# iyioon/NYPC-Yacht-Auction

Hardware: AMD Instinct MI355X
Metric: MCTS node-expansions/sec/GPU @4096 envs x100 sims; episodes/sec 1-8 GPU (higher is better)
Workload: dtype f32

## Files before the change

### include/yacht_hip.h

```cpp
#ifndef YACHT_HIP_H
#define YACHT_HIP_H

#include <stdint.h>

#ifdef __cplusplus
extern "C" {
#endif

#define YK_ACTION_SIZE 3226
#define YK_NUM_BID_ACTIONS 202
#define YK_FEATURES 59
#define YK_MASK_WORDS 101

typedef struct { uint64_t w[8]; } yk_state_t;

#define YK_OK 0
#define YK_ERR_ARG (-1)
#define YK_ERR_HIP (-2)
#define YK_ERR_NOMEM (-3)
#define YK_ERR_CAPACITY (-4)
#define YK_ERR_STATE (-5)
#define YK_ERR_RANGE (-6)

#define YK_ST_OK 0
// ... 64 lines not shown
                       void* stream);

typedef struct {
    int n_envs;
    int sims;
    double cpuct;
    int temp_threshold;
    int max_moves;
    int prior;
    int record_predictions;
    int max_expansions;
    int64_t arena_entries;
    int record_stride;
    int groups;
    int dual_trees;
    double dirichlet_alpha;
    double dirichlet_eps;
    int record_root_values;
} yk_engine_config_t;

typedef struct yk_engine yk_engine_t;
int yk_engine_create(yk_engine_t** eng, const yk_engine_config_t* cfg, yk_net_t* net);
int yk_engine_destroy(yk_engine_t* eng);
int yk_selfplay(yk_engine_t* eng, uint64_t seed, uint32_t env_base, void* stream);
int yk_engine_profile(yk_engine_t* eng, int enable);
int yk_engine_kernel_times(yk_engine_t* eng, double* ms, int64_t* launches);
int yk_engine_stats(yk_engine_t* eng, int64_t* out);
int yk_engine_counters(yk_engine_t* eng, int64_t* out, int n);
int yk_engine_records(yk_engine_t* eng, uint64_t* states, int32_t* info, uint64_t* ctr, double* values,
                      uint64_t* final_states, int32_t* n_moves, int64_t* visits_off, int32_t* visits,
                      int64_t* n_visits);
int yk_engine_predictions(yk_engine_t* eng, float* pi, float* v, yk_state_t* leaves, int32_t* count);
int yk_engine_root_priors(yk_engine_t* eng, float* before, float* after);
int yk_dirichlet_noise(uint64_t seed, const uint32_t* env_ids, const int32_t* moves, const int32_t* nvalid,
                       double alpha, double* eta, int n, void* stream);
int64_t yk_engine_record_bytes(yk_engine_t* eng);
int yk_engine_pack_records(yk_engine_t* eng, void* dst, int64_t capacity, void* stream);

int yk_examples_from_records(const void* images, int n_images, int n_envs, int max_moves, int sims,
                             int64_t n_games, int64_t skip, int64_t capacity, yk_state_t* states, int32_t* targets,
                             float* values, int64_t* n_examples, void* stream);
int yk_examples_policies(const void* images, int n_images, int n_envs, int max_moves, int sims, int64_t n_games,
                         int64_t skip, int64_t n_examples, int64_t* pi_indptr, int32_t* pi_cols, double* pi_vals,
                         int64_t nnz_capacity, double* values, int64_t* nnz, void* stream);
int yk_examples_value_targets(const void* images, int n_images, int n_envs, int max_moves, int sims,
                              int64_t n_games, int64_t skip, int64_t n_examples, double beta, double lambda,
                              float* values, float* root_values, int64_t* n_missing, void* stream);
#define YK_SYM_CARRY 1
#define YK_SYM_ROLLS 2
#define YK_SYM_GROUPS 4
int yk_examples_augment(const yk_state_t* states, const int32_t* targets, const int64_t* pi_indptr,
                        const int32_t* pi_cols, const double* pi_vals, int64_t n, int64_t index_base, uint64_t seed,
                        uint32_t epoch_key, int flags, yk_state_t* out_states, int32_t* out_targets,
                        int32_t* out_cols, double* out_vals, void* stream);

#define YK_PLAYER_MCTS 0
#define YK_PLAYER_RANDOM 1
#define YK_PLAYER_GREEDY 2
int yk_arena(yk_engine_t* eng, uint64_t seed, uint32_t env_base, const int32_t* agent_seat, int agent, int opponent,
             void* stream);
int yk_engine_set_opponent_net(yk_engine_t* eng, yk_net_t* net);
int yk_arena_results(yk_engine_t* eng, double* result, int32_t* totals, int32_t* n_moves, int32_t* actions,
                     uint64_t* final_states, uint64_t* rng_ctr);

int yk_mcts_search(yk_engine_t* eng, const yk_state_t* roots, uint64_t seed, const uint32_t* env_ids,
                   uint64_t* rng_ctr, int sims, int32_t* counts, void* stream);
// ... 44 lines not shown
```

### nypc-yacht-auction_amd/csrc/yk_engine.hip

```cpp
#include <math.h>

#include <algorithm>
#include <vector>

#include "yk_api.h"
#include "yk_common.h"
#include "yk_engine_dev.h"
#include "yk_net.h"

#define YK_MAX_GROUPS 8

using namespace yk;

namespace {


struct PwPlan {
    int nleaf, nop, root;
    uint16_t start[64], len[64];
    uint8_t a[64], b[64];
};
constexpr int pw_build(PwPlan& p, int start, int n) {
    if (n <= 128) {
        p.start[p.nleaf] = (uint16_t)start;
// ... 18 lines not shown
constexpr bool plan_is_butterfly() {
    const PwPlan p = make_plan();
    if (p.nleaf != 32 || p.nop != 31) return false;
    int first[128] = {}, cnt[128] = {};
    for (int i = 0; i < p.nleaf; i++) {
        if (p.start[i] % 8 != 0 || p.len[i] < 8 || p.len[i] > 128) return false;
        if (i > 0 && p.start[i] != p.start[i - 1] + p.len[i - 1]) return false;
        first[i] = i;
        cnt[i] = 1;
    }
    for (int o = 0; o < p.nop; o++) {
        const int a = p.a[o], b = p.b[o];
        if (cnt[a] != cnt[b] || first[a] + cnt[a] != first[b] || first[a] % (2 * cnt[a]) != 0) return false;
        first[64 + o] = first[a];
        cnt[64 + o] = 2 * cnt[a];
    }
    return p.root == 64 + p.nop - 1 && cnt[p.root] == 32;
}
static_assert(plan_is_butterfly(), "numpy's pairwise tree for 3226 is no longer a perfect 32-leaf tree");
constexpr int pw_gmax() {
    const PwPlan p = make_plan();
    int g = 0;
    for (int i = 0; i < p.nleaf; i++) g = p.len[i] / 8 > g ? p.len[i] / 8 : g;
    return g;
}
constexpr int pw_tmax() {
    const PwPlan p = make_plan();
    int t = 0;
    for (int i = 0; i < p.nleaf; i++) t = p.len[i] % 8 > t ? p.len[i] % 8 : t;
    return t;
}
constexpr int PW_GMAX = pw_gmax();
constexpr int PW_TMAX = pw_tmax() > 0 ? pw_tmax() : 1;

struct ValidQ {
    int mode;
    int n;
    uint32_t used;
    __device__ __forceinline__ bool operator()(int a) const {
        if (mode == 1) return a < NBID;
        if (mode != 0 || a < NBID) return false;
        const int base = a - NBID, cat = base / NCOMB, ci = base - cat * NCOMB;
        if ((used >> cat) & 1u) return false;
        if (n >= 10) return true;
        if (n == 5) return ci == 0;
        return c_tab.comb_max[ci] < n;
    }
};
__device__ __forceinline__ ValidQ valid_q(const YkS& s) {
    ValidQ q;
    const int round = s_round(s), phase = s_phase(s);
    const uint64_t wa = s_pw(s, 0, 0);
    q.n = __builtin_amdgcn_readfirstlane(wa_n(wa));
    q.used = __builtin_amdgcn_readfirstlane((uint32_t)wa_used(wa));
    q.mode = __builtin_amdgcn_readfirstlane((phase == 0 && round != 13) ? 1 : (phase == 1 && q.n >= 5) ? 0 : -1);
    return q;
}


__device__ __forceinline__ void wave_sync() {
    __builtin_amdgcn_fence(__ATOMIC_ACQ_REL, "workgroup");
    __builtin_amdgcn_wave_barrier();
}

__device__ __forceinline__ float wave_max(float v) {
    v = fmaxf(v, xlane<32>(v));
// ... 462 lines not shown
    const int t = __builtin_amdgcn_readfirstlane(tree_of(d, e));
    const int g = __builtin_amdgcn_readfirstlane((int)d.gen[t]);
    const bool idle = d.idle[e] != 0;
    expand_backup_game(d, e, lane, t, g);
    if (do_select) {
        if (idle) {
            select_none(d, e, lane);
            return;
        }
        wave_sync();
        select_game(d, e, lane, t, g, env_ids, ctr_arr);
    }
}

__device__ __forceinline__ void expand_backup_game(const EngDev& d, int e, int lane, int t, int g) {
    PyV res{d.res_v[e], d.res_t[e]};
    uint32_t end_id = 0;
    if (d.leaf_flag[e]) {
        const YkS s = ld_state(d.leaf_state + e);
        const uint64_t ihsh = d.leaf_hash[e];
        const uint64_t hsh = d.prior == 1 ? key_hash(s) : 0ull;
        const VInfo vi = valid_info(s, 1);
        const ValidQ valid = valid_q(s);
        const int V = vi.V;
        const int leaf = lane >> 1, h = lane & 1;
        const int st = c_pw.start[leaf], nl = c_pw.len[leaf], G = nl >> 3, R = nl & 7;
        float4 q[PW_GMAX];
        float qt[PW_TMAX];
        float v, mx = 0.f, lse = 0.f;
        const int pidx = (int)d.gstats[(long)e * GST + 0];
        const bool rec = d.rec_pred && (e % d.rec_stride) == 0 && pidx < d.max_exp;
        const long rslot = rec ? (long)(e / d.rec_stride) * d.max_exp + pidx : 0;
        bool masked = false;
        if (d.prior == 0) {
            const float* x = d.logits + (long)e * PI_LD + st;
            const float2 ml = d.mlse[e];
            mx = ml.x;
            lse = ml.y;
            if (d.fparts > 1) {
                float ms = ml.y;
                for (int p = 1; p < d.fparts; p++) {
                    const float2 q = d.mlse[(long)p * d.E + e];
                    const float mm = fmaxf(mx, q.x);
                    if (mm != -INFINITY) {
                        ms = ms * exp_acc(mx - mm) + q.y * exp_acc(q.x - mm);
                        mx = mm;
                    }
                }
                lse = logf(ms);
            }
            static_assert(NBID % 4 == 2 && NCOMB % 4 == 0, "category starts are 2 mod 4");
            const bool score10 = valid.mode == 0 && valid.n >= 10;
#pragma unroll
            for (int j = 0; j < PW_GMAX; j++) {
                const int a = st + 8 * j + 4 * h;
                bool v0, v1, v2, v3;
                if (score10) {
                    const int b0 = a - NBID, b2 = a + 2 - NBID;
                    const bool lo = j < G && b0 >= 0 && !((valid.used >> ((unsigned)b0 / NCOMB)) & 1u);
                    const bool hi = j < G && b2 >= 0 && !((valid.used >> ((unsigned)b2 / NCOMB)) & 1u);
                    v0 = v1 = lo;
                    v2 = v3 = hi;
                } else {
                    v0 = j < G && valid(a);
                    v1 = j < G && valid(a + 1);
                    v2 = j < G && valid(a + 2);
                    v3 = j < G && valid(a + 3);
                }
                float4 x4 = make_float4(0.f, 0.f, 0.f, 0.f);
                if (v0 || v1 || v2 || v3) x4 = *reinterpret_cast<const float4*>(x + 8 * j + 4 * h);
                q[j] = make_float4(v0 ? softmax_p(x4.x, mx, lse) : 0.f, v1 ? softmax_p(x4.y, mx, lse) : 0.f,
                                   v2 ? softmax_p(x4.z, mx, lse) : 0.f, v3 ? softmax_p(x4.w, mx, lse) : 0.f);
            }
#pragma unroll
            for (int r = 0; r < PW_TMAX; r++)
                qt[r] = (h == 0 && r < R && valid(st + 8 * G + r)) ? softmax_p(x[8 * G + r], mx, lse) : 0.f;
            v = d.vpred[e];
            masked = true;
        } else {
#pragma unroll
            for (int j = 0; j < PW_GMAX; j++) {
                const int a = st + 8 * j + 4 * h;
                q[j] = j < G ? make_float4(hash_prior_pi(hsh, a), hash_prior_pi(hsh, a + 1), hash_prior_pi(hsh, a + 2),
                                           hash_prior_pi(hsh, a + 3))
                             : make_float4(0.f, 0.f, 0.f, 0.f);
            }
#pragma unroll
            for (int r = 0; r < PW_TMAX; r++) qt[r] = (h == 0 && r < R) ? hash_prior_pi(hsh, st + 8 * G + r) : 0.f;
            v = hash_prior_v(hsh);
        }
#pragma unroll
        for (int j = 0; j < PW_GMAX; j++) {
            const int a = st + 8 * j + 4 * h;
            if (j < G && !masked) {
                if (!valid(a)) q[j].x = 0.f;
                if (!valid(a + 1)) q[j].y = 0.f;
                if (!valid(a + 2)) q[j].z = 0.f;
                if (!valid(a + 3)) q[j].w = 0.f;
            }
        }
#pragma unroll
        for (int r = 0; r < PW_TMAX; r++)
            if (h == 0 && r < R && !masked && !valid(st + 8 * G + r)) qt[r] = 0.f;
        if (rec) {
            float* rpi = d.rec_pi + rslot * ASIZE;
#pragma unroll
            for (int j = 0; j < PW_GMAX; j++)
                if (j < G) *reinterpret_cast<float4*>(rpi + st + 8 * j + 4 * h) = q[j];
#pragma unroll
            for (int r = 0; r < PW_TMAX; r++)
                if (h == 0 && r < R) rpi[st + 8 * G + r] = qt[r];
            if (lane == 0) {
                d.rec_v[rslot] = v;
                st_state(d.rec_leaf + rslot, s);
            }
        }
        float4 racc = q[0];
#pragma unroll
        for (int j = 1; j < PW_GMAX; j++)
            if (j < G) {
                racc.x += q[j].x;
                racc.y += q[j].y;
// ... 15 lines not shown
        lsum = (lane & 8) ? y + lsum : lsum + y;
        y = xlane<16>(lsum);
        lsum = (lane & 16) ? y + lsum : lsum + y;
        y = xlane<32>(lsum);
        lsum = (lane & 32) ? y + lsum : lsum + y;
        const float sum = lsum;
        const int VP = pad4(V);
        const uint32_t off = d.arena_top[t];
        const uint32_t nid = d.node_count[g * d.T + t];
        bool ok = true;
        if ((int64_t)off + VP > d.AE) {
            if (lane == 0) atomicOr(d.err, ERR_ARENA);
            ok = false;
        }
        if (nid >= (uint32_t)d.NCAP) {
            if (lane == 0) atomicOr(d.err, ERR_NODES);
            ok = false;
        }
        if (ok) {
            float* P = d.arenaP + (long)t * d.AE + off;
            uint16_t* S = d.arenaS + (long)t * d.AE + off;
            const float inv_fallback = V > 0 ? 1.0f / (float)V : 0.0f;
            const float* __restrict__ xr = d.logits + (long)e * PI_LD;
            const float sqe0 = (float)sqrt((double)0u + 1e-8);
            float fb = -INFINITY;
            int fj = 0x7FFFFFFF;
            for (int j0 = lane; j0 < VP; j0 += 256) {
                float xa[4];
                int aa[4];
#pragma unroll
                for (int u = 0; u < 4; u++) {
                    const int j = j0 + 64 * u;
                    aa[u] = j < V ? compact_to_action(vi, j) : 0;
                    xa[u] = (d.prior == 0 && j < V) ? xr[aa[u]] : 0.f;
                }
#pragma unroll
                for (int u = 0; u < 4; u++) {
                    const int j = j0 + 64 * u;
                    if (j < VP) {
                        float p = 0.0f;
                        if (j < V) {
                            const float pa = d.prior == 0 ? softmax_p(xa[u], mx, lse) : hash_prior_pi(hsh, aa[u]);
                            p = sum > 0.0f ? pa / sum : inv_fallback;
                            const float u0 = (d.c32 * p) * sqe0;
                            if (u0 > fb) {
                                fb = u0;
                                fj = j;
                            }
                        }
                        P[j] = p;
                        S[j] = 0;
                    }
                }
            }
            wave_argmax_step(fb, fj);
            if (lane == 0) {
                NodeRec r;
#pragma unroll
                for (int i = 0; i < 8; i++) r.key[i] = s.w[i];
                r.hash = ihsh;
                r.vinfo = pack_vinfo(vi);
                r.p_off = off;
                r.nvalid = (uint32_t)V;
                r.Ns = 0;
                r.first_j = (uint32_t)fj;
                d.nodes[g][(long)t * d.NCAP + nid] = r;
                if (!insert_index(d, g, t, ihsh, nid)) atomicOr(d.err, ERR_HASH);
            }
            end_id = nid + 1;
            if (lane == 0) {
                d.node_count[g * d.T + t] = nid + 1;
                d.arena_top[t] = off + (uint32_t)VP;
                unsigned long long* gs = reinterpret_cast<unsigned long long*>(d.gstats + (long)e * GST);
                atomicAdd(gs + 0, 1ull);
                atomicAdd(gs + 3, (unsigned long long)V);
                atomicMax(gs + 4, (unsigned long long)(nid + 1));
                atomicMax(gs + 6, (unsigned long long)(off + (uint32_t)VP));
            }
        }
        res = PyV{-(double)v, T_F32};
    } else {
        end_id = d.end_node[e];
    }
    const int depth = d.path_len[e];
    if (depth > 0) {
        NodeRec* nodes = d.nodes[g] + (long)t * d.NCAP;
        Edge* edges = d.edges[g] + (long)t * d.ECAP;
        uint16_t* Sb = d.arenaS + (long)t * d.AE;
        const uint64_t* path = d.path + (long)e * MAXD;
        const uint32_t ne0 = d.edge_count[g * d.T + t];
        uint64_t pe = 0;
        uint16_t sl = 0;
        if (lane < depth) {
            pe = path[lane];
            sl = Sb[pe >> 32];
        }
        const uint32_t pnext = __shfl((uint32_t)pe, (lane + 1) & 63, 64);
        const uint32_t cnode = lane + 1 < depth ? (pnext & ~PATH_DET) + 1 : end_id;
        const uint32_t cbits = ((uint32_t)pe & PATH_DET) ? cnode << 2 : 0u;
        const bool is_new = lane < depth && sl == 0;
        const uint64_t bal = __ballot(is_new);
        const uint32_t eid = ne0 + (uint32_t)__popcll(bal & ((1ull << lane) - 1));
        const uint32_t ne1 = ne0 + (uint32_t)__popcll(bal);
        if (lane < depth) {
            PyV v = res;
            if ((depth - 1 - lane) & 1) v.v = -v.v;
            if (sl) {
                Edge& ed = edges[sl - 1];
// ... 651 lines not shown
    A(d.idle, E);
    A(d.gstats, E * GST);
    A(d.err, 1);
    A(eng->done_count, 1);
    A(eng->mcts_env, E);
    if (d.prior == 0) {
        A(eng->logits, E * (size_t)PI_LD);
    }
    eng->root_values = cfg->record_root_values != 0;
    eng->noise = cfg->dirichlet_alpha > 0.0 && cfg->dirichlet_eps > 0.0;
    eng->nz.alpha = cfg->dirichlet_alpha;
    eng->nz.eps = cfg->dirichlet_eps;
    if (eng->noise) {
        A(eng->nz.noised, E);
        if (d.rec_pred) {
            A(eng->nz.prior_before, R * (size_t)d.M * ASIZE);
            A(eng->nz.prior_after, R * (size_t)d.M * ASIZE);
        }
    }
    if (d.rec_pred) {
        A(d.rec_pi, R * (size_t)d.max_exp * ASIZE);
        A(d.rec_v, R * (size_t)d.max_exp);
        A(d.rec_leaf, R * (size_t)d.max_exp);
    }
#undef A
    if (hipHostMalloc((void**)&eng->host_done, sizeof(int32_t)) != hipSuccess) return YK_ERR_NOMEM;
    {
        const char* ev = getenv("YK_ROOT_SCAN");
        eng->root_scan = !(ev && ev[0] == '0');
        const char* ek = getenv("YK_ROOT_K");
        d.ro_k = ek ? std::max(1, std::min(RO_K, atoi(ek))) : RO_K;
        const char* en = getenv("YK_NODE_SUMMARY");
        d.node_summary = (en && en[0] == '0') ? 0 : 1;
        const char* es = getenv("YK_SPLIT_DESCENT");
        eng->split_descent = es && es[0] == '1';
    }
    if (G > 1) {
        if (hipEventCreateWithFlags(&eng->ev_fork, hipEventDisableTiming) != hipSuccess) return YK_ERR_HIP;
        for (int g = 0; g < G; g++)
            if (hipStreamCreateWithFlags(&eng->gs[g], hipStreamNonBlocking) != hipSuccess ||
                hipEventCreateWithFlags(&eng->ev_join[g], hipEventDisableTiming) != hipSuccess ||
                hipEventCreateWithFlags(&eng->ev_fwd[g], hipEventDisableTiming) != hipSuccess)
                return YK_ERR_HIP;
    }
    if (eng->fparts_dual > 0) {
        if (hipStreamCreateWithFlags(&eng->dstream, hipStreamNonBlocking) != hipSuccess ||
            hipEventCreateWithFlags(&eng->ev_d0, hipEventDisableTiming) != hipSuccess ||
            hipEventCreateWithFlags(&eng->ev_d1, hipEventDisableTiming) != hipSuccess)
            return YK_ERR_HIP;
    }
    d.logits = eng->logits;
    d.vpred = eng->vpred;
    d.mlse = eng->mlse;
    d.lut_sq = eng->lut_sq;
    d.lut_sqe = eng->lut_sqe;
    hipLaunchKernelGGL(k_lut, dim3(LUT_N / 256), dim3(256), 0, 0, eng->lut_sq, eng->lut_sqe);
    YK_LAUNCHED();
    YK_HIP(hipMemset(d.err, 0, sizeof(uint32_t)));
    YK_HIP(hipMemset(d.done, 0, E));
    YK_HIP(hipMemset(d.idle, 0, E));
    YK_HIP(hipMemset(d.leaf_state, 0, sizeof(yk_state_t) * E));
    std::vector<uint32_t> ids(E);
    for (size_t i = 0; i < E; i++) ids[i] = (uint32_t)i;
    YK_HIP(hipMemcpy(eng->mcts_env, ids.data(), sizeof(uint32_t) * E, hipMemcpyHostToDevice));
    YK_HIP(hipDeviceSynchronize());
    *out = eng.release();
// ... 179 lines not shown
    YK_HIP(hipDeviceSynchronize());
    YK_HIP(hipMemcpy(gs.data(), d.gstats, sizeof(uint64_t) * gs.size(), hipMemcpyDeviceToHost));
    YK_HIP(hipMemcpy(nm.data(), d.nmoves, sizeof(int32_t) * nm.size(), hipMemcpyDeviceToHost));
    YK_HIP(hipMemcpy(&err, d.err, sizeof(uint32_t), hipMemcpyDeviceToHost));
    for (int i = 0; i < 16; i++) out[i] = 0;
    for (int e = 0; e < d.E; e++) {
        const uint64_t* g = &gs[(size_t)e * GST];
        out[0] += (int64_t)g[0];
        out[1] += (int64_t)g[1];
        out[2] = std::max<int64_t>(out[2], nm[e]);
        out[4] = std::max<int64_t>(out[4], (int64_t)g[4]);
        out[5] = std::max<int64_t>(out[5], (int64_t)g[5]);
        out[6] = std::max<int64_t>(out[6], (int64_t)g[6]);
        out[7] += (int64_t)g[3];
        out[8] += (int64_t)g[2];
        out[9] = std::max<int64_t>(out[9], (int64_t)g[7]);
    }
    out[3] = err;
    out[10] = d.NCAP;
    out[11] = d.ECAP;
    out[12] = d.AE;
    out[13] = d.VCAP;
    out[14] = eng->ngroups;
    out[15] = d.fparts;
    return YK_OK;
}

int yk_engine_counters(yk_engine_t* eng, int64_t* out, int n) {
    if (!eng || !out || n < 0) return YK_ERR_ARG;
    EngDev& d = eng->d;
    std::vector<uint64_t> gs((size_t)d.E * GST);
    YK_HIP(hipDeviceSynchronize());
    YK_HIP(hipMemcpy(gs.data(), d.gstats, sizeof(uint64_t) * gs.size(), hipMemcpyDeviceToHost));
    int64_t c[1] = {0};
    for (int e = 0; e < d.E; e++) c[0] += (int64_t)gs[(size_t)e * GST + 8];
    for (int i = 0; i < n; i++) out[i] = i < 1 ? c[i] : 0;
    return YK_OK;
}

int yk_engine_records(yk_engine_t* eng, uint64_t* states, int32_t* info, uint64_t* ctr, double* values,
                      uint64_t* final_states, int32_t* n_moves, int64_t* visits_off, int32_t* visits,
                      int64_t* n_visits) {
    if (!eng) return YK_ERR_ARG;
    if (!eng->have_records) return YK_ERR_STATE;
    EngDev& d = eng->d;
    const size_t E = d.E, M = d.M;
    YK_HIP(hipDeviceSynchronize());
    if (states) YK_HIP(hipMemcpy(states, d.rec_state, sizeof(yk_state_t) * E * M, hipMemcpyDeviceToHost));
    if (info) YK_HIP(hipMemcpy(info, d.rec_info, sizeof(int32_t) * E * M * 8, hipMemcpyDeviceToHost));
    if (ctr) YK_HIP(hipMemcpy(ctr, d.rec_ctr, sizeof(uint64_t) * E * M * 2, hipMemcpyDeviceToHost));
    if (values) YK_HIP(hipMemcpy(values, d.rec_val, sizeof(double) * E * M, hipMemcpyDeviceToHost));
    if (final_states) YK_HIP(hipMemcpy(final_states, d.board, sizeof(yk_state_t) * E, hipMemcpyDeviceToHost));
    if (n_moves) YK_HIP(hipMemcpy(n_moves, d.nmoves, sizeof(int32_t) * E, hipMemcpyDeviceToHost));
    if (visits_off || visits || n_visits) {
        std::vector<int32_t> voff(E * (M + 1));
        std::vector<int32_t> nm(E);
        YK_HIP(hipMemcpy(voff.data(), d.rec_voff, sizeof(int32_t) * voff.size(), hipMemcpyDeviceToHost));
        YK_HIP(hipMemcpy(nm.data(), d.nmoves, sizeof(int32_t) * E, hipMemcpyDeviceToHost));
        int64_t total = 0;
        for (size_t e = 0; e < E; e++) total += voff[e * (M + 1) + nm[e]];
        if (n_visits) *n_visits = total;
        if (visits_off || visits) {
            std::vector<uint32_t> raw(E * (size_t)d.VCAP);
            YK_HIP(hipMemcpy(raw.data(), d.rec_visits, sizeof(uint32_t) * raw.size(), hipMemcpyDeviceToHost));
            int64_t k = 0;
            for (size_t e = 0; e < E; e++) {
                for (size_t m = 0; m < M; m++) {
                    const int32_t a0 = voff[e * (M + 1) + m];
                    const int32_t a1 = (int)m < nm[e] ? voff[e * (M + 1) + m + 1] : a0;
// ... 9 lines not shown
            if (visits_off) visits_off[E * M] = k;
        }
    }
    return YK_OK;
}

int yk_engine_predictions(yk_engine_t* eng, float* pi, float* v, yk_state_t* leaves, int32_t* count) {
    if (!eng || !eng->d.rec_pred) return YK_ERR_ARG;
    EngDev& d = eng->d;
    const size_t R = ((size_t)d.E + d.rec_stride - 1) / d.rec_stride, X = (size_t)d.max_exp;
    YK_HIP(hipDeviceSynchronize());
    if (pi) YK_HIP(hipMemcpy(pi, d.rec_pi, sizeof(float) * R * X * ASIZE, hipMemcpyDeviceToHost));
    if (v) YK_HIP(hipMemcpy(v, d.rec_v, sizeof(float) * R * X, hipMemcpyDeviceToHost));
    if (leaves) YK_HIP(hipMemcpy(leaves, d.rec_leaf, sizeof(yk_state_t) * R * X, hipMemcpyDeviceToHost));
    if (count) {
        std::vector<uint64_t> gs((size_t)d.E * GST);
        YK_HIP(hipMemcpy(gs.data(), d.gstats, sizeof(uint64_t) * gs.size(), hipMemcpyDeviceToHost));
        for (size_t r = 0; r < R; r++) count[r] = (int32_t)gs[r * d.rec_stride * GST];
    }
    return YK_OK;
}

int yk_engine_root_priors(yk_engine_t* eng, float* before, float* after) {
    if (!eng) return YK_ERR_ARG;
    if (!eng->have_priors) return YK_ERR_STATE;
    EngDev& d = eng->d;
    const size_t n = (((size_t)d.E + d.rec_stride - 1) / d.rec_stride) * (size_t)d.M * ASIZE;
    YK_HIP(hipDeviceSynchronize());
    if (before) YK_HIP(hipMemcpy(before, eng->nz.prior_before, sizeof(float) * n, hipMemcpyDeviceToHost));
    if (after) YK_HIP(hipMemcpy(after, eng->nz.prior_after, sizeof(float) * n, hipMemcpyDeviceToHost));
    return YK_OK;
}

static void record_parts(yk_engine* eng, void** p, RecordLayout& L) {
    EngDev& d = eng->d;
    L = record_layout(d.E, d.M, d.VCAP);
    void* pp[REC_PARTS] = {d.rec_state, d.rec_info, d.rec_ctr, d.rec_val, d.rec_visits, d.rec_voff, d.nmoves, d.board};
    for (int i = 0; i < REC_PARTS; i++) p[i] = pp[i];
}

int64_t yk_engine_record_bytes(yk_engine_t* eng) {
    if (!eng) return YK_ERR_ARG;
    return record_layout(eng->d.E, eng->d.M, eng->d.VCAP).total;
}

int yk_engine_pack_records(yk_engine_t* eng, void* dst, int64_t capacity, void* stream) {
    if (!eng || !dst) return YK_ERR_ARG;
    if (!eng->have_records) return YK_ERR_STATE;
    void* p[REC_PARTS];
    RecordLayout L;
    record_parts(eng, p, L);
    if (capacity < L.total) return YK_ERR_ARG;
    for (int i = 0; i < REC_PARTS; i++)
        YK_HIP(hipMemcpyAsync((char*)dst + L.off[i], p[i], (size_t)L.bytes[i], hipMemcpyDeviceToDevice,
                              as_stream(stream)));
    return YK_OK;
}

int yk_mcts_reset(yk_engine_t* eng) {
    if (!eng) return YK_ERR_ARG;
    EngDev& d = eng->d;
    YK_HIP(hipMemset(d.err, 0, sizeof(uint32_t)));
    YK_HIP(hipMemset(d.hidx[0], 0, sizeof(uint32_t) * (size_t)d.T * d.HCAP));
    YK_HIP(hipMemset(d.done, 0, (size_t)d.E));
    hipLaunchKernelGGL(k_reset, dim3((d.E + 255) / 256), dim3(256), 0, 0, d, 0, 0u);
    YK_LAUNCHED();
// ... 25 lines not shown
```

### nypc-yacht-auction_amd/csrc/yk_engine_dev.h

```cpp
#pragma once
#include <math.h>
#include <stddef.h>

#include <type_traits>

#include "yk_api.h"
#include "yk_common.h"

using namespace yk;

namespace {

constexpr int MAXD = 64;
constexpr int LUT_N = 1 << 16;
constexpr int GAMES_PER_BLOCK = 4;
constexpr int GROUP_ALIGN = 16;
constexpr int YK_EXPAND_WPE = 4;
constexpr int RO_CAP = 3072;
constexpr int RO_K = 512;
constexpr int RV_CAP = 1024;
constexpr uint32_t RV_OFF = 0xFFFFFFFFu;

enum : uint32_t { T_INT = 0, T_F64 = 1, T_F32 = 2 };

struct NodeRec {
    uint64_t key[8];
    uint64_t hash;
    uint64_t vinfo;
    uint32_t p_off;
    uint32_t nvalid;
    uint32_t Ns;
    uint32_t first_j;
};
static_assert(sizeof(NodeRec) == 96, "NodeRec: 96 bytes");
struct Edge {
    double Q;
    uint32_t N;
    uint32_t tag;
};
__device__ __forceinline__ uint32_t edge_kind(uint32_t tag) { return tag & 3u; }
constexpr uint32_t PATH_DET = 0x80000000u;

constexpr int GST = 16;
struct EngDev {
    int E, NCAP, HCAP, ECAP, M, VCAP;
    int e_lo, e_hi;
    int T, dual;
    int64_t AE;
    int sims, temp_threshold;
    float c32;
    int prior;
    int fparts;
    int rec_pred, max_exp, rec_stride;
    int arena;
    int arena_agent, arena_opp;
    uint64_t seed;
    NodeRec* nodes[2];
    uint32_t* hidx[2];
    Edge* edges[2];
    uint32_t* node_count;
    uint32_t* edge_count;
    float* arenaP;
    uint16_t* arenaS;
    uint32_t* arena_top;
    uint8_t* gen;
    uint8_t* cur_round;
    uint4* root_c;
    int node_summary;
    int ro_k;
    uint32_t* rv;
    uint16_t* ro_j;
    float* ro_p;
    yk_state_t* board;
    int32_t* cur;
    uint64_t* ctr;
    uint32_t* env_id;
    uint8_t* done;
    int32_t* nmoves;
    yk_state_t* root;
    int32_t* seat;
    uint8_t* idle;
    yk_state_t* leaf_state;
    uint64_t* leaf_hash;
    uint8_t* leaf_flag;
    uint64_t* path;
    uint8_t* path_len;
    uint32_t* end_node;
    double* res_v;
    uint32_t* res_t;
    const float* logits;
    const float* vpred;
    const float2* mlse;
    const float* lut_sq;
    const float* lut_sqe;
    yk_state_t* rec_state;
    int32_t* rec_info;
    uint64_t* rec_ctr;
    double* rec_val;
    uint32_t* rec_visits;
    int32_t* rec_voff;
    double* final_r;
// ... 145 lines not shown
```

### nypc-yacht-auction_amd/yacht_amd/_lib.py

```python
from __future__ import annotations

import ctypes as C
import os
import subprocess

HERE = os.path.dirname(os.path.abspath(__file__))
PKG_ROOT = os.path.dirname(HERE)
LIB_PATH = os.environ.get("YK_LIB_PATH") or os.path.join(HERE, "libyacht_hip.so")

YK_OK, YK_ERR_ARG, YK_ERR_HIP, YK_ERR_NOMEM, YK_ERR_CAPACITY, YK_ERR_STATE = 0, -1, -2, -3, -4, -5
YK_ERR_RANGE = -6
_ERR_NAMES = {YK_ERR_ARG: "bad argument", YK_ERR_HIP: "HIP error", YK_ERR_NOMEM: "out of device memory",
              YK_ERR_CAPACITY: "engine capacity exceeded", YK_ERR_STATE: "engine state error",
              YK_ERR_RANGE: "a value outside the range the operation accepts (a net weight with |w| >= 65520, "
                            "the fp16 split's range; sampling weights negative, NaN or without a finite positive total; "
                            "splice rows not strictly ascending within the CSR)"}
YK_NET_ERR_SYNC = 1

ST_OK, ST_VALUE_BID, ST_VALUE_SCORE, ST_RUNTIME, ST_ASSERT, ST_CAPACITY = 0, 1, 2, 3, 4, 5


class YkError(RuntimeError):
    def __init__(self, fn, code):
        hip = _lib.yk_last_hip_error() if _lib is not None else 0
# ... 39 lines not shown
    "yk_net_destroy": [P],
    "yk_net_set_precision": [P, I],
    "yk_net_errors": [P, P],
    "yk_engine_create": [C.POINTER(P), C.POINTER(YkEngineConfig), P],
    "yk_engine_destroy": [P],
    "yk_selfplay": [P, U64, U32, P],
    "yk_arena": [P, U64, U32, P, I, I, P],
    "yk_greedy_action": [P, P, I, P],
    "yk_trainer_create": [P, I, I, P, I, P],
    "yk_trainer_destroy": [P],
    "yk_trainer_buffers": [P, P, P, P],
    "yk_trainer_backward": [P, P, P, P, P, I, P],
    "yk_trainer_apply": [P, P],
    "yk_trainer_step": [P, P, P, P, P, I, P],
    "yk_trainer_backward_soft": [P, P, P, P, P, P, P, I, P],
    "yk_trainer_step_soft": [P, P, P, P, P, P, P, I, P],
    "yk_trainer_losses": [P, P],
    "yk_trainer_epoch_loss_begin": [P, C.c_double],
    "yk_trainer_epoch_loss_end": [P, P],
    "yk_trainer_get": [P, I, P],
    "yk_trainer_set": [P, I, P, C.c_int64],
    "yk_trainer_step_count": [P],
    "yk_trainer_set_row_offset": [P, C.c_int64],
    "yk_trainer_amp_state": [P, P],
    "yk_arena_results": [P, P, P, P, P, P, P],
    "yk_engine_set_opponent_net": [P, P],
    "yk_engine_stats": [P, P],
    "yk_engine_counters": [P, P, I],
    "yk_engine_profile": [P, I],
    "yk_engine_kernel_times": [P, P, P],
    "yk_engine_records": [P, P, P, P, P, P, P, P, P, P],
    "yk_engine_predictions": [P, P, P, P, P],
    "yk_engine_root_priors": [P, P, P],
    "yk_dirichlet_noise": [U64, P, P, P, C.c_double, P, I, P],
    "yk_engine_record_bytes": [P],
    "yk_engine_pack_records": [P, P, C.c_int64, P],
    "yk_mcts_search": [P, P, U64, P, P, I, P, P],
    "yk_mcts_reset": [P],
    "yk_examples_from_records": [P, I, I, I, I, C.c_int64, C.c_int64, C.c_int64, P, P, P, P, P],
    "yk_examples_policies": [P, I, I, I, I, C.c_int64, C.c_int64, C.c_int64, P, P, P, C.c_int64, P, P, P],
    "yk_examples_augment": [P, P, P, P, P, C.c_int64, C.c_int64, U64, U32, I, P, P, P, P, P],
    "yk_examples_value_targets": [P, I, I, I, I, C.c_int64, C.c_int64, C.c_int64, C.c_double, C.c_double, P, P, P, P],
    "yk_net_logits": [P, P, P, P, I, P],
    "yk_examples_metrics": [P, C.c_int64, P, P, P, P, P, P, P, P, C.c_int64, P, P, P],
    "yk_net_evaluate": [P, P, P, P, P, P, P, P, C.c_int64, I, P, P, P],
    "yk_sample_weights": [P, C.c_int64, P, P, I, C.c_double, C.c_int64, P, P, P],
    "yk_sample_cdf": [P, C.c_int64, P, P, P],
    "yk_sample_draw": [P, C.c_int64, U64, U32, U64, C.c_int64, P, P],
    "yk_reanalyse_select": [C.c_int64, U64, U64, U32, C.c_double, P, C.c_int64, P, P],
    "yk_policies_from_counts": [P, C.c_int64, P, P, P, C.c_int64, P, P, P, P],
    "yk_policies_splice": [P, P, P, C.c_int64, P, C.c_int64, P, P, P, P, P, P, C.c_int64, P, P],
}
_RESTYPE = {"yk_version": C.c_char_p, "yk_rng_draw64": C.c_uint64, "yk_engine_record_bytes": C.c_int64,
            "yk_trainer_step_count": C.c_int64}

_NEWER = {"yk_engine_counters", "yk_net_errors", "yk_trainer_backward_soft", "yk_trainer_step_soft",
          "yk_engine_root_priors", "yk_dirichlet_noise", "yk_examples_augment", "yk_examples_value_targets",
          "yk_net_logits", "yk_examples_metrics", "yk_net_evaluate", "yk_sample_weights", "yk_sample_cdf",
          "yk_sample_draw", "yk_reanalyse_select", "yk_policies_from_counts", "yk_policies_splice"}
_lib = None


def build() -> str:
    subprocess.run(["make", "-C", PKG_ROOT, "-j4"], check=True)
    return LIB_PATH


def lib():
    global _lib
    if _lib is None:
        if not os.path.exists(LIB_PATH):
            raise ImportError(f"{LIB_PATH} not found: build it with `make -C {PKG_ROOT}` "
                              "(or __graft_entry__.build()); there is no CPU fallback")
        lib_ = C.CDLL(LIB_PATH)
        for name, args in SIGNATURES.items():
            if os.environ.get("YK_LIB_PATH") and name in _NEWER and not hasattr(lib_, name):
                continue
            fn = getattr(lib_, name)
            fn.argtypes = args
            fn.restype = _RESTYPE.get(name, C.c_int)
        _lib = lib_
    return _lib


def call(name, *args):
    rc = getattr(lib(), name)(*args)
    if rc != YK_OK:
        raise YkError(name, rc)
    return rc


def ptr(t) -> int:
# ... 12 lines not shown
```

### nypc-yacht-auction_amd/yacht_amd/engine.py

```python
from __future__ import annotations

import ctypes as C

import numpy as np
import torch

from ._lib import YkEngineConfigFull, call, lib, stream_ptr

ACTION_SIZE = 3226


class SelfPlayEngine:
    def __init__(self, n_envs: int, sims: int, cpuct: float = 1.5, temp_threshold: int = 15, net=None,
                 prior: str = "net", max_moves: int = 64, record_predictions: bool = False,
                 max_expansions: int = 0, arena_entries: int = 0, record_stride: int = 1, groups: int = 0,
                 dual_trees: bool = False, opponent_net=None, dirichlet_alpha: float = 0.0,
                 dirichlet_eps: float = 0.0, record_root_values: bool = False):
        if prior not in ("net", "hash"):
            raise ValueError("prior is 'net' (YachtNNet on MFMA) or 'hash' (deterministic test prior)")
        if prior == "net" and net is None:
            raise ValueError("prior='net' needs a YkNet")
        self.cfg = YkEngineConfigFull(
            n_envs=n_envs, sims=sims, cpuct=cpuct, temp_threshold=temp_threshold,
            max_moves=max_moves, prior=0 if prior == "net" else 1,
# ... 40 lines not shown
            raise YkError(f"yk_arena [{', '.join(bits)}; stats {st}]", e.code) from None

    def arena_results(self) -> dict:
        E, M = self.n_envs, self.max_moves
        result = np.zeros(E, dtype=np.float64)
        totals = np.zeros((E, 2), dtype=np.int32)
        nm = np.zeros(E, dtype=np.int32)
        actions = np.zeros((E, M), dtype=np.int32)
        final = np.zeros((E, 8), dtype=np.uint64)
        ctr = np.zeros(E, dtype=np.uint64)
        call("yk_arena_results", self.handle, result.ctypes.data, totals.ctypes.data, nm.ctypes.data,
             actions.ctypes.data, final.ctypes.data, ctr.ctypes.data)
        return dict(result=result, totals=totals, n_moves=nm, actions=actions, final=final, ctr=ctr)

    KERNEL_CLASSES = ("select", "forward", "root_sort_select", "expand_backup_select", "move_begin", "move_end")

    def profile(self, enable: bool = True, stride: int = 1):
        call("yk_engine_profile", self.handle, int(stride) if enable else 0)

    def kernel_times(self) -> dict:
        ms = np.zeros(8, dtype=np.float64)
        n = np.zeros(8, dtype=np.int64)
        call("yk_engine_kernel_times", self.handle, ms.ctypes.data, n.ctypes.data)
        kt = {k: (float(ms[i]), int(n[i])) for i, k in enumerate(self.KERNEL_CLASSES) if k != "unused"}
        if self.cfg.dirichlet_alpha > 0 and self.cfg.dirichlet_eps > 0:
            kt["root_noise"] = (float(ms[6]), int(n[6]))
        if self.cfg.record_root_values:
            kt["root_value"] = (float(ms[7]), int(n[7]))
        return kt

    STAT_NAMES = ("expansions", "scanned", "moves", "errors", "max_nodes", "max_edges", "max_arena", "vnew",
                  "path_edges", "sims", "node_cap", "edge_cap", "arena_cap", "visit_cap", "groups",
                  "forward_parts")
    COUNTER_NAMES = ("scan_edges",)

    def stats(self) -> dict:
        out = np.zeros(16, dtype=np.int64)
        call("yk_engine_stats", self.handle, out.ctypes.data)
        st = {k: int(out[i]) for i, k in enumerate(self.STAT_NAMES)}
        more = np.zeros(len(self.COUNTER_NAMES), dtype=np.int64)
        if hasattr(lib(), "yk_engine_counters"):
            call("yk_engine_counters", self.handle, more.ctypes.data, len(more))
        st.update({k: int(more[i]) for i, k in enumerate(self.COUNTER_NAMES)})
        return st

    def records(self) -> dict:
        E, M = self.n_envs, self.max_moves
        states = np.zeros((E, M, 8), dtype=np.uint64)
        info = np.zeros((E, M, 8), dtype=np.int32)
        ctr = np.zeros((E, M, 2), dtype=np.uint64)
        values = np.zeros((E, M), dtype=np.float64)
        final = np.zeros((E, 8), dtype=np.uint64)
        nm = np.zeros(E, dtype=np.int32)
        nv = np.zeros(1, dtype=np.int64)
        call("yk_engine_records", self.handle, None, None, None, None, None, None, None, None, nv.ctypes.data)
        voff = np.zeros(E * M + 1, dtype=np.int64)
        visits = np.zeros((max(int(nv[0]), 1), 2), dtype=np.int32)
        call("yk_engine_records", self.handle, states.ctypes.data, info.ctypes.data, ctr.ctypes.data,
             values.ctypes.data, final.ctypes.data, nm.ctypes.data, voff.ctypes.data, visits.ctypes.data,
             nv.ctypes.data)
        rec = dict(states=states, info=info, ctr=ctr, values=values, final=final, n_moves=nm,
                   visits_off=voff.reshape(-1)[:E * M + 1], visits=visits[:int(nv[0])])
        if self.cfg.record_root_values:
            rec["root_values"] = decode_root_values(info[:, :, 7])
        return rec

    def predictions(self, leaves: bool = False):
# ... 63 lines not shown
```

Baseline: 31.26 million.

## Scatter valid-action priors into shared-memory window before pairwise sum in expansion

The leaf-expansion kernel gets a fast path. It gathers softmax priors only for the valid actions, scatters them into a per-wave shared-memory window (a dense span, or one slot per category in the five-dice case), and feeds the pairwise-sum layout from that window. This replaces masked float4 loads over the full 3226-action logits row, and the later normalisation pass reuses the window instead of reloading logits and recomputing softmax. It costs up to 32KB of LDS per block plus extra wave syncs, and it adds a debug root-prior export and counters.

```diff
diff --git a/include/yacht_hip.h b/include/yacht_hip.h
--- a/include/yacht_hip.h
+++ b/include/yacht_hip.h
@@ -120,6 +120,7 @@
                       int64_t* n_visits);
 int yk_engine_predictions(yk_engine_t* eng, float* pi, float* v, yk_state_t* leaves, int32_t* count);
 int yk_engine_root_priors(yk_engine_t* eng, float* before, float* after);
+int yk_engine_root_prior(yk_engine_t* eng, int game, float* p);
 int yk_dirichlet_noise(uint64_t seed, const uint32_t* env_ids, const int32_t* moves, const int32_t* nvalid,
                        double alpha, double* eta, int n, void* stream);
 int64_t yk_engine_record_bytes(yk_engine_t* eng);
diff --git a/nypc-yacht-auction_amd/csrc/yk_engine.hip b/nypc-yacht-auction_amd/csrc/yk_engine.hip
--- a/nypc-yacht-auction_amd/csrc/yk_engine.hip
+++ b/nypc-yacht-auction_amd/csrc/yk_engine.hip
@@ -74,6 +74,15 @@
 }
 constexpr int PW_GMAX = pw_gmax();
 constexpr int PW_TMAX = pw_tmax() > 0 ? pw_tmax() : 1;
+constexpr int pw_lmax() {
+    const PwPlan p = make_plan();
+    int l = 0;
+    for (int i = 0; i < p.nleaf; i++) l = p.len[i] > l ? p.len[i] : l;
+    return l;
+}
+static_assert(NCOMB > pw_lmax(), "two category starts could share a leaf of the pairwise plan");
+static_assert(PF_WCAP % 8 == 0 && PF_WCAP >= 16 && GAMES_PER_BLOCK * PF_WCAP * 4 <= 40 * 1024,
+              "the prior window: whole float4 pairs, a slot per category, 16 waves per CU");
 
 struct ValidQ {
     int mode;
@@ -602,8 +611,23 @@
         const bool rec = d.rec_pred && (e % d.rec_stride) == 0 && pidx < d.max_exp;
         const long rslot = rec ? (long)(e / d.rec_stride) * d.max_exp + pidx : 0;
         bool masked = false;
+        __shared__ __attribute__((aligned(16))) float s_win[GAMES_PER_BLOCK][PF_WCAP];
+        float* win = s_win[threadIdx.x >> 6];
+        int fast = 0, wbase = 0, wlen = 0;
+        if (d.prior_fast && V > 0) {
+            if (valid.mode == 0 && valid.n == 5) {
+                fast = 2;
+                wlen = 16;
+            } else {
+                const int a0 = __builtin_amdgcn_readfirstlane(compact_to_action(vi, 0));
+                const int a1 = __builtin_amdgcn_readfirstlane(compact_to_action(vi, V - 1));
+                wbase = a0 & ~7;
+                wlen = (a1 + 1 - wbase + 7) & ~7;
+                fast = wlen <= PF_WCAP ? 1 : 0;
+            }
+        }
+        const auto wslot = [&](int a) { return fast == 2 ? (a - NBID) / NCOMB : a - wbase; };
         if (d.prior == 0) {
-            const float* x = d.logits + (long)e * PI_LD + st;
             const float2 ml = d.mlse[e];
             mx = ml.x;
             lse = ml.y;
@@ -619,6 +643,69 @@
                 }
                 lse = logf(ms);
             }
+            v = d.vpred[e];
+        } else {
+            v = hash_prior_v(hsh);
+        }
+        if (fast) {
+            for (int i = 4 * lane; i < wlen; i += 256) *reinterpret_cast<float4*>(win + i) = make_float4(0.f, 0.f, 0.f, 0.f);
+            wave_sync();
+            const float* __restrict__ xr = d.logits + (long)e * PI_LD;
+            for (int j0 = lane; j0 < V; j0 += 256) {
+                float xa[4];
+                int aa[4];
+#pragma unroll
+                for (int u = 0; u < 4; u++) {
+                    const int j = j0 + 64 * u;
+                    aa[u] = j < V ? compact_to_action(vi, j) : 0;
+                    xa[u] = (d.prior == 0 && j < V) ? xr[aa[u]] : 0.f;
+                }
+#pragma unroll
+                for (int u = 0; u < 4; u++)
+                    if (j0 + 64 * u < V)
+                        win[wslot(aa[u])] = d.prior == 0 ? softmax_p(xa[u], mx, lse) : hash_prior_pi(hsh, aa[u]);
+            }
+            wave_sync();
+            int soff = -8;
+            float4 sv = make_float4(0.f, 0.f, 0.f, 0.f);
+            if (fast == 2) {
+                const int c = st <= NBID ? 0 : (st - NBID + NCOMB - 1) / NCOMB;
+                const int o = NBID + NCOMB * c - st;
+                if (c < NCAT && o < nl) {
+                    const float pc = win[c];
+                    soff = o;
+                    sv = make_float4((o & 3) == 0 ? pc : 0.f, (o & 3) == 1 ? pc : 0.f, (o & 3) == 2 ? pc : 0.f,
+                                     (o & 3) == 3 ? pc : 0.f);
+                }
+            }
+#pragma unroll
+            for (int j = 0; j < PW_GMAX; j++) {
+                const int o = 8 * j + 4 * h;
+                float4 w = make_float4(0.f, 0.f, 0.f, 0.f);
+                if (fast == 1) {
+                    const int i = st + o - wbase;
+                    if (j < G && (unsigned)i < (unsigned)wlen) w = *reinterpret_cast<const float4*>(win + i);
+                } else if (j < G && o == (soff & ~3)) {
+                    w = sv;
+                }
+                q[j] = w;
+            }
+#pragma unroll
+            for (int r = 0; r < PW_TMAX; r++) {
+                const int o = 8 * G + r, i = st + o - wbase;
+                float w = 0.f;
+                if (h == 0 && r < R) {
+                    if (fast == 1) {
+                        if ((unsigned)i < (unsigned)wlen) w = win[i];
+                    } else if (o == soff) {
+                        w = win[wslot(st + o)];
+                    }
+                }
+                qt[r] = w;
+            }
+            masked = true;
+        } else if (d.prior == 0) {
+            const float* x = d.logits + (long)e * PI_LD + st;
             static_assert(NBID % 4 == 2 && NCOMB % 4 == 0, "category starts are 2 mod 4");
             const bool score10 = valid.mode == 0 && valid.n >= 10;
 #pragma unroll
@@ -645,7 +732,6 @@
 #pragma unroll
             for (int r = 0; r < PW_TMAX; r++)
                 qt[r] = (h == 0 && r < R && valid(st + 8 * G + r)) ? softmax_p(x[8 * G + r], mx, lse) : 0.f;
-            v = d.vpred[e];
             masked = true;
         } else {
 #pragma unroll
@@ -657,7 +743,6 @@
             }
 #pragma unroll
             for (int r = 0; r < PW_TMAX; r++) qt[r] = (h == 0 && r < R) ? hash_prior_pi(hsh, st + 8 * G + r) : 0.f;
-            v = hash_prior_v(hsh);
         }
 #pragma unroll
         for (int j = 0; j < PW_GMAX; j++) {
@@ -739,7 +824,7 @@
                 for (int u = 0; u < 4; u++) {
                     const int j = j0 + 64 * u;
                     aa[u] = j < V ? compact_to_action(vi, j) : 0;
-                    xa[u] = (d.prior == 0 && j < V) ? xr[aa[u]] : 0.f;
+                    xa[u] = (d.prior == 0 && !fast && j < V) ? xr[aa[u]] : 0.f;
                 }
 #pragma unroll
                 for (int u = 0; u < 4; u++) {
@@ -747,7 +832,9 @@
                     if (j < VP) {
                         float p = 0.0f;
                         if (j < V) {
-                            const float pa = d.prior == 0 ? softmax_p(xa[u], mx, lse) : hash_prior_pi(hsh, aa[u]);
+                            const float pa = fast            ? win[wslot(aa[u])]
+                                             : d.prior == 0 ? softmax_p(xa[u], mx, lse)
+                                                            : hash_prior_pi(hsh, aa[u]);
                             p = sum > 0.0f ? pa / sum : inv_fallback;
                             const float u0 = (d.c32 * p) * sqe0;
                             if (u0 > fb) {
@@ -781,6 +868,7 @@
                 unsigned long long* gs = reinterpret_cast<unsigned long long*>(d.gstats + (long)e * GST);
                 atomicAdd(gs + 0, 1ull);
                 atomicAdd(gs + 3, (unsigned long long)V);
+                atomicAdd(gs + (fast == 1 ? 9 : fast == 2 ? 10 : 11), 1ull);
                 atomicMax(gs + 4, (unsigned long long)(nid + 1));
                 atomicMax(gs + 6, (unsigned long long)(off + (uint32_t)VP));
             }
@@ -1498,6 +1586,8 @@
         d.ro_k = ek ? std::max(1, std::min(RO_K, atoi(ek))) : RO_K;
         const char* en = getenv("YK_NODE_SUMMARY");
         d.node_summary = (en && en[0] == '0') ? 0 : 1;
+        const char* ep = getenv("YK_PRIOR_FAST");
+        d.prior_fast = (ep && ep[0] == '0') ? 0 : 1;
         const char* es = getenv("YK_SPLIT_DESCENT");
         eng->split_descent = es && es[0] == '1';
     }
@@ -1743,9 +1833,12 @@
     std::vector<uint64_t> gs((size_t)d.E * GST);
     YK_HIP(hipDeviceSynchronize());
     YK_HIP(hipMemcpy(gs.data(), d.gstats, sizeof(uint64_t) * gs.size(), hipMemcpyDeviceToHost));
-    int64_t c[1] = {0};
-    for (int e = 0; e < d.E; e++) c[0] += (int64_t)gs[(size_t)e * GST + 8];
-    for (int i = 0; i < n; i++) out[i] = i < 1 ? c[i] : 0;
+    int64_t c[4] = {0, 0, 0, 0};
+    for (int e = 0; e < d.E; e++) {
+        c[0] += (int64_t)gs[(size_t)e * GST + 8];
+        for (int k = 0; k < 3; k++) c[1 + k] += (int64_t)gs[(size_t)e * GST + 9 + k];
+    }
+    for (int i = 0; i < n; i++) out[i] = i < 4 ? c[i] : 0;
     return YK_OK;
 }
 
@@ -1821,6 +1914,28 @@
     return YK_OK;
 }
 
+int yk_engine_root_prior(yk_engine_t* eng, int game, float* p) {
+    if (!eng || !p || game < 0 || game >= eng->d.E) return YK_ERR_ARG;
+    EngDev& d = eng->d;
+    uint4 rc[2];
+    YK_HIP(hipDeviceSynchronize());
+    YK_HIP(hipMemcpy(rc, d.root_c + 2 * game, sizeof(rc), hipMemcpyDeviceToHost));
+    if (rc[0].x == 0) return YK_ERR_STATE;
+    const uint64_t x = (uint64_t)rc[1].x | ((uint64_t)rc[1].y << 32);
+    VInfo vi;
+    vi.cats = x & 0xFFFFFFFFFFFFull;
+    vi.k = (int)((x >> 48) & 0xF);
+    vi.n = (int)((x >> 52) & 0xF);
+    vi.W = (int)(x >> 56);
+    vi.V = (int)rc[0].z;
+    std::vector<float> P((size_t)vi.V);
+    if (vi.V > 0)
+        YK_HIP(hipMemcpy(P.data(), d.arenaP + (size_t)game * d.AE + rc[0].y, sizeof(float) * P.size(), hipMemcpyDeviceToHost));
+    for (int a = 0; a < ASIZE; a++) p[a] = 0.f;
+    for (int j = 0; j < vi.V; j++) p[compact_to_action(vi, j)] = P[j];
+    return YK_OK;
+}
+
 static void record_parts(yk_engine* eng, void** p, RecordLayout& L) {
     EngDev& d = eng->d;
     L = record_layout(d.E, d.M, d.VCAP);
diff --git a/nypc-yacht-auction_amd/csrc/yk_engine_dev.h b/nypc-yacht-auction_amd/csrc/yk_engine_dev.h
--- a/nypc-yacht-auction_amd/csrc/yk_engine_dev.h
+++ b/nypc-yacht-auction_amd/csrc/yk_engine_dev.h
@@ -20,6 +20,7 @@
 constexpr int RO_K = 512;
 constexpr int RV_CAP = 1024;
 constexpr uint32_t RV_OFF = 0xFFFFFFFFu;
+constexpr int PF_WCAP = 2048;
 
 enum : uint32_t { T_INT = 0, T_F64 = 1, T_F32 = 2 };
 
@@ -67,6 +68,7 @@
     uint8_t* cur_round;
     uint4* root_c;
     int node_summary;
+    int prior_fast;
     int ro_k;
     uint32_t* rv;
     uint16_t* ro_j;
diff --git a/nypc-yacht-auction_amd/yacht_amd/_lib.py b/nypc-yacht-auction_amd/yacht_amd/_lib.py
--- a/nypc-yacht-auction_amd/yacht_amd/_lib.py
+++ b/nypc-yacht-auction_amd/yacht_amd/_lib.py
@@ -95,6 +95,7 @@
     "yk_engine_records": [P, P, P, P, P, P, P, P, P, P],
     "yk_engine_predictions": [P, P, P, P, P],
     "yk_engine_root_priors": [P, P, P],
+    "yk_engine_root_prior": [P, I, P],
     "yk_dirichlet_noise": [U64, P, P, P, C.c_double, P, I, P],
     "yk_engine_record_bytes": [P],
     "yk_engine_pack_records": [P, P, C.c_int64, P],
@@ -120,7 +121,8 @@
 _NEWER = {"yk_engine_counters", "yk_net_errors", "yk_trainer_backward_soft", "yk_trainer_step_soft",
           "yk_engine_root_priors", "yk_dirichlet_noise", "yk_examples_augment", "yk_examples_value_targets",
           "yk_net_logits", "yk_examples_metrics", "yk_net_evaluate", "yk_sample_weights", "yk_sample_cdf",
-          "yk_sample_draw", "yk_reanalyse_select", "yk_policies_from_counts", "yk_policies_splice"}
+          "yk_sample_draw", "yk_reanalyse_select", "yk_policies_from_counts", "yk_policies_splice",
+          "yk_engine_root_prior"}
 _lib = None
 
 
diff --git a/nypc-yacht-auction_amd/yacht_amd/engine.py b/nypc-yacht-auction_amd/yacht_amd/engine.py
--- a/nypc-yacht-auction_amd/yacht_amd/engine.py
+++ b/nypc-yacht-auction_amd/yacht_amd/engine.py
@@ -96,7 +96,7 @@
     STAT_NAMES = ("expansions", "scanned", "moves", "errors", "max_nodes", "max_edges", "max_arena", "vnew",
                   "path_edges", "sims", "node_cap", "edge_cap", "arena_cap", "visit_cap", "groups",
                   "forward_parts")
-    COUNTER_NAMES = ("scan_edges",)
+    COUNTER_NAMES = ("scan_edges", "prior_window", "prior_sparse", "prior_general")
 
     def stats(self) -> dict:
         out = np.zeros(16, dtype=np.int64)
```

Result: faster. 32.02 million (median of 6 runs) (+2.4%).
